# elucideye/acf

Measured on AMD Instinct MI355X. Metric: detector FPS @1080p, 8 scales/octave, FACE80 model, higher is better.
Workload: dtype f32

## Files before the change

### acf_amd/capi.py

```python
import ctypes as C
import os

import numpy as np

_HERE = os.path.dirname(os.path.abspath(__file__))
LIB_PATH = os.environ.get("ACF_HIP_LIB") or os.path.join(_HERE, "libacf_hip.so")

OK = 0
E_INVALID, E_UNSUPPORTED, E_NOMODEL, E_NOPLAN, E_HIP, E_NODEVICE, E_CAPACITY = 1, 2, 3, 4, 5, 6, 7
NMS_CAP = 2048
CS_GRAY, CS_RGB, CS_LUV, CS_HSV, CS_ORIG = 0, 1, 2, 3, 4
TAP_IMAGE, TAP_SMOOTHED, TAP_M, TAP_O, TAP_S, TAP_MNORM, TAP_CHNS, TAP_LDCF = range(8)


class Params(C.Structure):

    _fields_ = [
        ("nTrees", C.c_int32),
        ("nTreeNodes", C.c_int32),
        ("treeDepth", C.c_int32),
        ("fids", C.POINTER(C.c_uint32)),
        ("thrs", C.POINTER(C.c_float)),
        ("hs", C.POINTER(C.c_float)),
        ("child", C.POINTER(C.c_uint32)),
# ... 153 lines not shown
    fp = C.POINTER(C.c_float)
    sig = {
        "acf_hip_create": ([C.c_int, C.c_void_p, C.POINTER(ctx)], C.c_int),
        "acf_hip_destroy": ([ctx], C.c_int),
        "acf_hip_abi_version": ([], C.c_int),
        "acf_hip_device_count": ([C.POINTER(C.c_int)], C.c_int),
        "acf_hip_last_error": ([ctx], C.c_char_p),
        "acf_hip_set_option": ([ctx, C.c_char_p, C.c_int], C.c_int),
        "acf_hip_set_model": ([ctx, C.POINTER(Params)], C.c_int),
        "acf_hip_get_scales": ([C.c_int] * 7 + [C.POINTER(C.c_double)] * 3 + [C.c_int, C.POINTER(C.c_int)], C.c_int),
        "acf_hip_plan_levels": ([C.POINTER(Params), C.c_int, C.c_int, C.c_int, C.POINTER(Level), C.c_int, C.POINTER(C.c_int), C.POINTER(C.c_int)], C.c_int),
        "acf_hip_plan": ([ctx, C.c_int, C.c_int, C.c_int, C.c_int, C.c_int], C.c_int),
        "acf_hip_num_levels": ([ctx, C.POINTER(C.c_int), C.POINTER(C.c_int)], C.c_int),
        "acf_hip_get_levels": ([ctx, C.POINTER(Level), C.c_int], C.c_int),
        "acf_hip_get_ldcf_levels": ([ctx, C.POINTER(Level), C.c_int], C.c_int),
        "acf_hip_pyramid_floats": ([ctx, C.POINTER(C.c_int64)], C.c_int),
        "acf_hip_get_lambdas": ([ctx, C.c_int, C.POINTER(C.c_double)], C.c_int),
        "acf_hip_pyramid": ([ctx, C.c_void_p, C.c_int], C.c_int),
        "acf_hip_detect": ([ctx], C.c_int),
        "acf_hip_run": ([ctx, C.c_void_p, C.c_int], C.c_int),
        "acf_hip_run_host": ([ctx, fp, C.c_int], C.c_int),
        "acf_hip_pyramid_u8": ([ctx, C.c_void_p, C.c_int, C.c_int, C.c_int], C.c_int),
        "acf_hip_run_u8": ([ctx, C.c_void_p, C.c_int, C.c_int, C.c_int], C.c_int),
        "acf_hip_pyramid_image": ([ctx, C.c_void_p, C.c_int, C.POINTER(ImageDesc)], C.c_int),
        "acf_hip_run_image": ([ctx, C.c_void_p, C.c_int, C.POINTER(ImageDesc)], C.c_int),
        "acf_hip_image_extent": ([C.POINTER(ImageDesc), C.c_int, C.c_int, C.c_int, C.POINTER(C.c_int64), C.POINTER(C.c_int64)], C.c_int),
        "acf_hip_pyramid_yuv": ([ctx, C.c_void_p, C.c_int, C.POINTER(YuvDesc)], C.c_int),
        "acf_hip_run_yuv": ([ctx, C.c_void_p, C.c_int, C.POINTER(YuvDesc)], C.c_int),
        "acf_hip_yuv_to_rgb8": ([ctx, C.c_void_p, C.c_int, C.c_int, C.c_int, C.POINTER(YuvDesc), C.c_void_p], C.c_int),
        "acf_hip_yuv_extent": ([C.POINTER(YuvDesc), C.c_int, C.c_int, C.c_int, C.POINTER(C.c_int64), C.POINTER(C.c_int64)], C.c_int),
# ... 49 lines not shown
    return lib


DECLARED_SYMBOLS = [
    "acf_hip_create", "acf_hip_device_count", "acf_hip_destroy", "acf_hip_abi_version", "acf_hip_last_error", "acf_hip_set_option",
    "acf_hip_set_model", "acf_hip_get_scales", "acf_hip_plan_levels",
    "acf_hip_plan", "acf_hip_num_levels", "acf_hip_get_levels", "acf_hip_get_ldcf_levels", "acf_hip_pyramid_floats", "acf_hip_get_lambdas", "acf_hip_pyramid",
    "acf_hip_detect", "acf_hip_run", "acf_hip_run_host", "acf_hip_set_nms", "acf_hip_op_nms", "acf_hip_get_detections", "acf_hip_get_hits", "acf_hip_get_raw_detections",
    "acf_hip_pyramid_u8", "acf_hip_run_u8", "acf_hip_set_yuv_layout", "acf_hip_op_yuv420_to_rgb", "acf_hip_u8_frame_bytes", "acf_hip_resize_dims", "acf_hip_set_input_resize", "acf_hip_op_resize_u8", "acf_hip_stream_open", "acf_hip_stream_submit", "acf_hip_stream_collect",
    "acf_hip_stream_close", "acf_hip_host_alloc", "acf_hip_host_free",
    "acf_hip_export_detections", "acf_hip_synchronize", "acf_hip_get_repairs", "acf_hip_profile_get", "acf_hip_read_level", "acf_hip_read_rank_level", "acf_hip_rank_cells_host", "acf_hip_read_tap",
    "acf_hip_op_rgb_convert", "acf_hip_op_conv_tri", "acf_hip_op_gradient_mag", "acf_hip_selftest_gradmag", "acf_hip_set_x86_tables", "acf_hip_selftest_x86", "acf_hip_chns_compute", "acf_hip_op_gradient_hist",
    "acf_hip_op_im_resample", "acf_hip_op_acf_detect1", "acf_hip_op_acf_detect1_u8", "acf_hip_thrs_u8", "acf_hip_op_evaluate",
    "acf_hip_evaluate_crops", "acf_hip_evaluate_crops_u8",
    "acf_hip_pyramid_image", "acf_hip_run_image", "acf_hip_image_extent",
    "acf_hip_pyramid_yuv", "acf_hip_run_yuv", "acf_hip_yuv_to_rgb8", "acf_hip_yuv_extent", "acf_hip_yuv_layout", "acf_hip_stream_open_yuv",
]


def fptr(a):
    return a.ctypes.data_as(C.POINTER(C.c_float))
```

### acf_amd/csrc/acf_hip.hip

```cpp
#include "kernels.hip.h"

#include <algorithm>
#include <cmath>
#include <cstdio>
#include <cstring>
#include <functional>
#include <mutex>
#include <string>
#include <type_traits>
#include <vector>

using namespace acfhip;

namespace
{

struct DevBuf
{
    void* p = nullptr;
    size_t bytes = 0;
};

struct ResampleTiling
{
// ... 18 lines not shown
    StripPlan strip, stripPair;
    float *img = nullptr, *sm = nullptr, *M = nullptr, *O = nullptr, *U = nullptr, *S = nullptr, *Mn = nullptr;
    int64_t uFloats = 0, moFloats = 0;
};

}

struct TileSet
{
    bool ok = false;
    TileGeom g{};
    int nTiles = 0, aTB = 4;
    CascTile* d_tiles = nullptr;
    TreeNode* d_tileNodes = nullptr;
    uint32_t* d_tileNodesS = nullptr;
    uint32_t* d_nodesD = nullptr;
    int tbD = 0, t1D = 0;
    uint32_t* d_tileOffD = nullptr;
    uint32_t* d_thrsRankD = nullptr;
};

struct LeafCodes
{
    uint8_t* d = nullptr;
    int cap = 0, pitch = 0;
};

struct QueueCounters
{
    static constexpr size_t TILE_COUNTERS = 8;
// ... 260 lines not shown
{
    FB_TRIY_UNFUSED = 1u << 0,
    FB_MOU_PLAIN = 1u << 1,
    FB_RESAMPLE_NO_STRIP = 1u << 2,
    FB_RESAMPLE_NO_PAIR = 1u << 3,
    FB_RESAMPLE_NO_UP = 1u << 4,
    FB_RESAMPLE_GENERIC = 1u << 5,
    FB_LEVEL_GROUPS = 1u << 6,
    FB_LDCF_UNFUSED = 1u << 7,
    FB_NO_DEDUP = 1u << 8,
    FB_NO_TAIL_CODES = 1u << 9,
    FB_TAIL3 = 1u << 10,
    FB_TILED_STAGED = 1u << 11,
    FB_TILED_POOLED1 = 1u << 12,
    FB_YUV_UNFUSED = 1u << 13,
};
uint32_t fallbackMask()
{
    static const uint32_t mask = [] {
        static const struct { const char* name; uint32_t bit; } kNames[] = {
            { "triy_unfused", FB_TRIY_UNFUSED }, { "mou_plain", FB_MOU_PLAIN }, { "resample_no_strip", FB_RESAMPLE_NO_STRIP },
            { "resample_no_pair", FB_RESAMPLE_NO_PAIR }, { "resample_no_up", FB_RESAMPLE_NO_UP }, { "resample_generic", FB_RESAMPLE_GENERIC },
            { "level_groups", FB_LEVEL_GROUPS }, { "ldcf_unfused", FB_LDCF_UNFUSED }, { "no_dedup", FB_NO_DEDUP }, { "no_tail_codes", FB_NO_TAIL_CODES },
            { "tail3", FB_TAIL3 }, { "tiled_staged", FB_TILED_STAGED }, { "tiled_pooled1", FB_TILED_POOLED1 },
            { "yuv_unfused", FB_YUV_UNFUSED } };
        uint32_t m = 0;
        const char* e = getenv("ACF_HIP_FORCE_FALLBACK");
        std::string s = e ? e : "";
        size_t i = 0;
        while (i < s.size())
        {
            size_t j = s.find(',', i);
            j = j == std::string::npos ? s.size() : j;
            const std::string tok = s.substr(i, j - i);
            bool known = tok.empty();
            for (const auto& n : kNames)
            {
                if (tok == n.name)
                {
                    m |= n.bit;
// ... 1198 lines not shown
    }
    return ACF_HIP_OK;
}

int acf_hip_get_levels(const acf_hip_ctx* c, acf_hip_level* out, int cap)
{
    if (int rc = needPlanRead(c, "get_levels")) return rc;
    if (!out || cap < int(c->plan.levels.size()))
    {
        return fail(c, ACF_HIP_E_INVALID, "get_levels: capacity");
    }
    std::copy(c->plan.levels.begin(), c->plan.levels.end(), out);
    return ACF_HIP_OK;
}

int acf_hip_get_ldcf_levels(const acf_hip_ctx* c, acf_hip_level* out, int cap)
{
    if (!c || !c->hasPlan || !out)
    {
        return ACF_HIP_E_INVALID;
    }
    const acf_hip_ctx* src = c->kids.empty() ? c : c->kids[0];
    if (src->p.ldcfK <= 0 || src->ldcf.levels.empty())
    {
        return ACF_HIP_E_INVALID;
    }
    const int n = std::min(cap, int(src->ldcf.levels.size()));
    std::copy(src->ldcf.levels.begin(), src->ldcf.levels.begin() + n, out);
    return ACF_HIP_OK;
}
// ... 1266 lines not shown
```

### acf_amd/csrc/cascade_plan.hip.h

```cpp
#pragma once

struct FeatPos
{
    uint32_t z, cc, rr;
};

static inline FeatPos splitFid(uint32_t f, int mW, int mH)
{
    return { f / uint32_t(mW * mH), (f / uint32_t(mH)) % uint32_t(mW), f % uint32_t(mH) };
}

static size_t pooledTileLds(const TileGeom& g, int cellBytes, size_t leafBytes)
{
    const size_t nwin = size_t(g.NW) * 64;
    return leafBytes + size_t(g.tileFloats) * cellBytes + ((std::max(nwin * 8, size_t(g.passW) * size_t(g.pitchC)) + 15) / 16 * 16) + nwin * 8;
}

static int buildTileSet(acf_hip_ctx* c, const CascState& cs, const std::vector<float>& thrs, const std::vector<acf_hip_level>& lv, int nChns, const RankTables* rank,
    TileSet& out, bool allowPooledD = true)
{
    const acf_hip_params& p = c->p;
    const int mH = p.modelDsPad_h / cs.cell, mW = p.modelDsPad_w / cs.cell;
    const int cellBytes = rank ? 2 : 4, CPB = 16 / cellBytes;
    int rc;
// ... 95 lines not shown
    g.colsT = (g.TC - 1) * g.step + mW;
    g.rowsP = (g.rowsT + CPB - 1) / CPB * CPB;
    g.tileFloats = nChns * g.rowsP * g.colsT;
    g.cpsMagic = uint32_t(((uint64_t(1) << 32) + uint32_t(g.rowsP / CPB) - 1) / uint32_t(g.rowsP / CPB));
    g.colsMagic = uint32_t(((uint64_t(1) << 32) + uint32_t(g.colsT) - 1) / uint32_t(g.colsT));
    std::vector<CascTile> tiles;
    bool ok = true;
    {
        const uint32_t cps = uint32_t(g.rowsP / CPB), nSeg = uint32_t(nChns * g.colsT);
        for (uint32_t q = 0; q < nSeg * cps && ok; q++)
        {
            const uint32_t seg = uint32_t((uint64_t(q) * g.cpsMagic) >> 32);
            ok = seg == q / cps && uint32_t((uint64_t(seg) * g.colsMagic) >> 32) == seg / uint32_t(g.colsT);
        }
    }
    for (size_t i = 0; i < lv.size() && ok; i++)
    {
        for (int c0 = 0; c0 < lv[i].nWinC; c0 += g.TC)
        {
            for (int r0 = 0; r0 < lv[i].nWinR; r0 += g.TR)
            {
                if (r0 > 32767 || c0 > 32767)
                {
                    ok = false;
                    break;
                }
                CascTile t{};
                t.level = int16_t(i);
                t.r0 = int16_t(r0);
                t.c0 = int16_t(c0);
                tiles.push_back(t);
            }
        }
    }
    if (!ok)
    {
        return ACF_HIP_OK;
    }
    if (p.treeDepth != 2)
    {
        const int D = p.treeDepth;
        if ((rank && !g.pooled) || D < 1 || D > 4 || D == 2)
        {
            return ACF_HIP_OK;
        }
        const int NN = (1 << D) - 1, NL = 1 << D, TB = D == 1 ? 4 : (D == 3 ? 2 : 1);
        const int t1 = std::min(32, p.nTrees) / TB * TB;
// ... 48 lines not shown
            {
                return rc;
            }
        }
        out.g = g;
        out.nTiles = int(tiles.size());
        out.tbD = TB;
        out.t1D = t1;
        if ((rc = devUpload(c, &out.d_nodesD, nd)) || (rc = devUpload(c, &out.d_tiles, tiles)))
        {
            return rc;
        }
        out.ok = true;
        return ACF_HIP_OK;
    }
    std::vector<TreeNode> tileNodes(size_t(std::max(p.nTrees, 1)));
    for (int t = 0; t < p.nTrees; t++)
    {
        const size_t q = size_t(t) * p.nTreeNodes;
        TreeNode a{};
        for (int k = 0; k < 3; k++)
        {
            const FeatPos f = splitFid(c->fids[q + k], mW, mH);
            a.off[k] = (f.z * uint32_t(g.colsT) + f.cc) * uint32_t(g.rowsP) + f.rr;
            if (rank)
            {
                const uint32_t rk = rank->rankOfThreshold(int(f.z), thrs[q + k]);
                memcpy(&a.thr[k], &rk, 4);
            }
            else
            {
                a.thr[k] = thrs[q + k];
            }
        }
        for (int k = 0; k < 4; k++)
        {
            a.hs[k] = c->hs[q + 3 + k];
        }
        tileNodes[size_t(t)] = a;
    }
    const int aTB = 4;
    const int nTreesS = (g.pooled ? g.b[2] : g.b[1]) / aTB * aTB;
    std::vector<uint32_t> nodesS(size_t(std::max(nTreesS / aTB, 1)) * 10 * aTB, 0u);
    for (int t = 0; t + aTB - 1 < nTreesS; t += aTB)
    {
        uint32_t* d = nodesS.data() + size_t(t / aTB) * 10 * aTB;
        for (int q = 0; q < aTB; q++)
        {
            const TreeNode& nd = tileNodes[size_t(t + q)];
            for (int k = 0; k < 3; k++)
            {
                d[3 * q + k] = nd.off[k];
                memcpy(&d[3 * aTB + 3 * q + k], &nd.thr[k], 4);
            }
            for (int k = 0; k < 4; k++)
            {
                memcpy(&d[6 * aTB + 4 * q + k], &nd.hs[k], 4);
            }
        }
    }
    out.aTB = aTB;
    out.g = g;
    out.nTiles = int(tiles.size());
    if ((rc = devUpload(c, &out.d_tileNodesS, nodesS)) || (rc = devUpload(c, &out.d_tiles, tiles)) || (rc = devUpload(c, &out.d_tileNodes, tileNodes)))
    {
        return rc;
    }
    out.ok = true;
    return ACF_HIP_OK;
}

static LeafCodes leafCodeBuffer(acf_hip_ctx* c, const std::vector<acf_hip_level>& lv, int nT, int batch)
{
    LeafCodes lc;
    lc.pitch = (nT + 63) / 64 * 64;
    int64_t nWinTotal = 0;
    for (const auto& l : lv)
    {
// ... 357 lines not shown
```

### acf_amd/csrc/cascade_run.hip.h

```cpp
#pragma once

extern "C++"
{
template <class Args>
static int launchLds(acf_hip_ctx* c, void (*kernel)(Args), dim3 grid, dim3 block, size_t lds, const Args& a)
{
    int rc;
    if ((rc = allowLds(c, reinterpret_cast<const void*>(kernel), lds)))
    {
        return rc;
    }
    hipLaunchKernelGGL(kernel, grid, block, lds, c->stream, a);
    return ACF_HIP_OK;
}
}

using TileKernel = void (*)(TileArgs);
using TileDKernel = void (*)(TileDArgs);
using CascKernel = void (*)(CascArgs);

static TileKernel tile3Kernel(int nw, bool rank)
{
    if (rank)
    {
// ... 313 lines not shown
    {
        a.mH = c->p.modelDsPad_h / cs.cell;
        a.mW = c->p.modelDsPad_w / cs.cell;
    }
}
}

static void setTiles(TileArgs& a, const TileSet& ts)
{
    a.g = ts.g;
    a.tiles = ts.d_tiles;
    a.nTiles = ts.nTiles;
    a.tileNodes = ts.d_tileNodes;
    a.tileNodesS = ts.d_tileNodesS;
    a.aTB = ts.aTB;
}

static TileArgs tiled2Args(const acf_hip_ctx* c, const CascState& cs, const CascadeCall& call)
{
    const QueueCounters qc = cs.counters();
    TileArgs a{};
    fillShared(a, c, cs, call);
    setTiles(a, cs.tiles);
    a.nTrees = c->p.nTrees;
    a.tailNodes = cs.d_tailNodes;
    a.q = cs.d_queue[0];
    a.qcount = qc.queueCount();
    a.qhead = qc.queueHead();
    a.tileNext = qc.tileNext2();
    a.tailScratch = cs.d_tailScratch;
// ... 399 lines not shown
```

### acf_amd/csrc/host_plan.cpp

```cpp
#include "host_plan.h"

#include <algorithm>
#include <cfloat>
#include <cmath>
#include <cstring>
#include <limits>

namespace acfhip
{

ScaleList getScales(int nPerOct, int nOctUp, int minDs_h, int minDs_w, int shrink, int H, int W)
{
    ScaleList out;
    if (H <= 0 || W <= 0)
    {
        return out;
    }
    const double szw = H, szh = W;
    const double ratio_w = szw / double(minDs_h), ratio_h = szh / double(minDs_w);
    const double lg = std::log(std::min(ratio_w, ratio_h)) / std::log(2.0);
    const int nScales = int(std::floor(double(nPerOct) * (double(nOctUp) + lg) + 1.0));
    double d0 = szh, d1 = szw;
    if (szh >= szw)
    {
// ... 740 lines not shown
    {
        t.xlin[size_t(dx) * 4 + 3] = dx < xmax ? 1 : 0;
    }
    for (int dy = 0; dy < t.drows; dy++)
    {
        float f = float((dy + 0.5) * sc - 0.5);
        const int sy = cvFloorD(f);
        f -= sy;
        t.ylin[size_t(dy) * 4] = std::min(std::max(sy, 0), rows - 1);
        t.ylin[size_t(dy) * 4 + 1] = std::min(std::max(sy + 1, 0), rows - 1);
        t.ylin[size_t(dy) * 4 + 2] = satS16((1.f - f) * 2048.f);
        t.ylin[size_t(dy) * 4 + 3] = satS16(f * 2048.f);
    }
    return 0;
}
}
```

### acf_amd/csrc/host_plan.h

```cpp
#pragma once

#include "../../include/acf_hip.h"

#include <cstdint>
#include <string>
#include <vector>

namespace acfhip
{

struct ScaleList
{
    std::vector<double> scales, shw_h, shw_w;
};

ScaleList getScales(int nPerOct, int nOctUp, int minDs_h, int minDs_w, int shrink, int H, int W);

struct AxisCoef
{
    int na = 0, nb = 0;
    bool down = false;
    int bd[2] = { 0, 0 };
    std::vector<int> start;
    std::vector<int> src;
// ... 88 lines not shown
};

void buildRankTables(const float* thrs, const int32_t* chnOfNode, size_t nNodes, int nChns, RankTables& out);

struct ResizeTables
{
    int rows = 0, cols = 0, drows = 0, dcols = 0;
    int mode = 0, isx = 1, isy = 1;
    std::vector<int32_t> xlin, ylin;
    std::vector<int32_t> xrun, yrun;
    std::vector<int32_t> xtap, ytap;
};
void resizeDims(int rows, int cols, double scale, int& drows, int& dcols);
int buildResizeTables(int rows, int cols, double scale, ResizeTables& t);

int colorPlanes(const acf_hip_params& p);
int numChannels(const acf_hip_params& p);
int numChannels(const acf_hip_params& p, int dcol);

}
```

### acf_amd/csrc/kernels_cascade.hip.h

```cpp
#pragma once

namespace acfhip
{

struct CascLevel
{
    int32_t hP, wP, nWinR, nWinC;
    int32_t firstBlock;
    int32_t nWin;
    int64_t off;
    int64_t nodeOff;
    int64_t offR;
    int32_t pitchR;
    int32_t padR_;
};

struct __attribute__((aligned(16))) CascNode2
{
    uint32_t zcr[4];
    float thr[4];
    float hs[4];
};

struct CascArgs
// ... 476 lines not shown
            acf_hip_hit hit;
            hit.scale = lvl;
            hit.c = n / nWinR;
            hit.r = n - hit.c * nWinR;
            hit.score = h;
            a.hits[int64_t(frame) * a.maxHits + idx] = hit;
        }
    }
}

typedef uint32_t u32x4 __attribute__((ext_vector_type(4)));
typedef const __attribute__((address_space(4))) u32x4* cptr4_t;

struct CascTile
{
    int16_t level, pad_;
    int16_t r0, c0;
};

static_assert(sizeof(CascTile) == 8, "k_cascade_tile3 reads a CascTile as two dwords");
static_assert(offsetof(CascLevel, nWinR) == 8 && offsetof(CascLevel, off) == 24 && offsetof(CascLevel, offR) == 40 && offsetof(CascLevel, pitchR) == 48,
    "k_cascade_tile3 reads a CascLevel as dwords");

typedef const __attribute__((address_space(4))) uint32_t* cu32_k;
__device__ __forceinline__ CascTile load_tile_k(const CascTile* p)
{
    cu32_k tp = (cu32_k)(uintptr_t)p;
    const uint32_t w0 = tp[0], w1 = tp[1];
    CascTile T;
    T.level = int16_t(w0 & 0xffffu);
    T.pad_ = 0;
    T.r0 = int16_t(w1 & 0xffffu);
    T.c0 = int16_t(w1 >> 16);
    return T;
}
__device__ __forceinline__ CascLevel load_level_k(const CascLevel* p)
{
    cu32_k lp = (cu32_k)(uintptr_t)p;
    CascLevel L;
    L.hP = int32_t(lp[0]);
    L.wP = int32_t(lp[1]);
    L.nWinR = int32_t(lp[2]);
    L.nWinC = int32_t(lp[3]);
    L.off = int64_t(uint64_t(lp[6]) | (uint64_t(lp[7]) << 32));
    L.offR = int64_t(uint64_t(lp[10]) | (uint64_t(lp[11]) << 32));
    L.pitchR = int32_t(lp[12]);
// ... 8 lines not shown
};

struct TileGeom
{
    int32_t TR, TC, NW, W;
    int32_t step;
    int32_t rowsT, colsT;
    int32_t rowsP;
    int32_t tileFloats;
    uint32_t cpsMagic, colsMagic;
    int32_t b[5];
    int32_t winFloats;
    int32_t pooled;
    int32_t passW;
    int32_t pitchC;
};

struct TileArgs
{
    const float* pyr;
    int64_t pyr_fs;
    const uint16_t* pyrR;
    int64_t pyrR_fs;
    const CascLevel* levels;
    const CascTile* tiles;
    int32_t nTiles, nFrames, nChns, mH, mW, nTrees;
    TileGeom g;
    const TreeNode* tileNodes;
    const uint32_t* tileNodesS;
    int32_t aTB;
// ... 2 lines not shown
    uint2* q;
    int32_t* qcount;
    int32_t* qhead;
    int32_t* tileNext;
    int32_t qcap;
    acf_hip_hit* hits;
    int32_t* counts;
    int32_t maxHits;
    int32_t debug;
    long long* stamps;
    float* tailScratch;
    int32_t tailPad, tailSlab;
    int32_t tailNodesLds;
    uint8_t* tailCodes;
    int32_t codeCap, codePitch;
};

struct LaneNode
{
    uint4 o, tq, hq;
};

#ifdef ACF_HIP_STAMPS
#define TILE_STAMP(k)                                                          \
    if ((a.debug & 4) && threadIdx.x == 0)                                      \
    {                                                                          \
        a.stamps[int64_t(blockIdx.x) * 8 + (k)] = __builtin_amdgcn_s_memtime(); \
    }
#else
#define TILE_STAMP(k)
// ... 221 lines not shown
    }
    alive = alive && (hMin > thrC);
}

template <int NW, class CT>
__global__ void __launch_bounds__(NW * 64) k_cascade_tile3(TileArgs a)
{
    typedef typename CT::cell_t cell_t;
    typedef typename CT::val_t val_t;
    constexpr int CPB = CT::CPB;
    constexpr int NT = NW * 64;
    extern __shared__ float lds[];
    __shared__ int s_n[4];
    float* leafT = lds;
    cell_t* tileF = reinterpret_cast<cell_t*>(reinterpret_cast<char*>(lds) + TILE3_LEAF_BYTES);
    const int NWIN = a.g.TR * a.g.TC;
    char* r1 = reinterpret_cast<char*>(tileF) + size_t(a.g.tileFloats) * sizeof(cell_t);
    const int passW = a.g.passW;
    const int r1Bytes = (max(NWIN * 8, passW * a.g.pitchC) + 15) & ~15;
    uint2* l1 = reinterpret_cast<uint2*>(r1);
    uint8_t* codes = reinterpret_cast<uint8_t*>(r1);
    uint2* l2 = reinterpret_cast<uint2*>(r1 + r1Bytes);
    const int tid = threadIdx.x, lane = tid & 63, wv = tid >> 6;

    const int64_t total = int64_t(a.nTiles) * a.nFrames;
    const int perX = int((total + 7) >> 3);
    const int xcd = blockIdx.x & 7;
    __shared__ int s_next[2];
    const bool persist = a.tileNext != nullptr;
    int li = int(blockIdx.x >> 3);
    if (persist)
    {
        if (tid == 0)
        {
            s_next[0] = atomicAdd(a.tileNext + xcd, 1);
        }
        __syncthreads();
        li = __builtin_amdgcn_readfirstlane(s_next[0]);
    }
    int par = 1;
    const int step = a.g.step, rowsP = a.g.rowsP, TR = a.g.TR;
    const int b1 = a.g.b[1], b2 = a.g.b[2], tEnd = a.g.b[4];
    const int Ts = tEnd - b2, TsPad = (Ts + 15) & ~15;
    const int tlShift = TsPad <= 32 ? 5 : (TsPad <= 64 ? 6 : 7);
    const int pos = tid & ((1 << tlShift) - 1);
    uint32_t so0 = 0, so1 = 0, so2 = 0, st0 = 0, st1 = 0, st2 = 0;
    if (Ts > 0)
    {
        const uint4* np = reinterpret_cast<const uint4*>(a.tileNodes + b2 + min(pos, Ts - 1));
        const uint4 o = np[0], tq = np[1];
        so0 = o.x, so1 = o.y, so2 = o.z;
        st0 = tq.x, st1 = tq.y, st2 = tq.z;
    }
    bool leavesDone = Ts <= 0;
    for (;;)
    {
    const int64_t id = int64_t(xcd) * perX + li;
    if (li >= perX || id >= total)
    {
        break;
    }
    int liNext = perX;
    if (tid == 0 && persist)
    {
        liNext = atomicAdd(a.tileNext + xcd, 1);
    }
    const int frame = int(id / a.nTiles);
    const CascTile T = load_tile_k(a.tiles + (id - int64_t(frame) * a.nTiles));
    const int lvl = T.level;
    const CascLevel L = load_level_k(a.levels + lvl);
    const int nWinR = L.nWinR;
    if (tid < 4)
    {
        s_n[tid] = 0;
    }
    TILE_STAMP(0);
    {
        const int colsT = a.g.colsT;
        const int gr0 = T.r0 * step, gc0 = T.c0 * step;
        const int colPitch = CT::RANK ? L.pitchR : L.hP;
        const int area = colPitch * L.wP;
        const cell_t* __restrict__ src0 = (CT::RANK ? reinterpret_cast<const cell_t*>(a.pyrR) + int64_t(frame) * a.pyrR_fs + L.offR
                                                    : reinterpret_cast<const cell_t*>(a.pyr) + int64_t(frame) * a.pyr_fs + L.off) + gr0;
        const srd_t fsrd = make_srd(src0, int64_t(a.nChns) * area * int64_t(sizeof(cell_t)));
        const int colsValid = min(colsT, L.wP - gc0);
        const uint32_t cps = uint32_t(rowsP) / uint32_t(CPB);
        const uint32_t nChunks = uint32_t(a.nChns * colsT) * cps;
        const int ccMax = colsValid - 1;
        for (uint32_t q0 = uint32_t(wv) * 64u; q0 < nChunks; q0 += NW * 64u)
        {
            const uint32_t q = q0 + lane;
            if (q < nChunks)
            {
                const uint32_t seg = __umulhi(q, a.g.cpsMagic);
                const uint32_t j = q - seg * cps;
                const uint32_t z = __umulhi(seg, a.g.colsMagic);
                const int cc = int(seg - z * uint32_t(colsT));
                const uint32_t soff = z * uint32_t(area) + uint32_t(gc0 + min(cc, ccMax)) * uint32_t(colPitch) + uint32_t(CPB) * j;
                __builtin_amdgcn_raw_ptr_buffer_load_lds(fsrd, (lptr_t)(tileF + uint32_t(CPB) * q0), 16, soff * uint32_t(sizeof(cell_t)), 0, 0, 0);
            }
        }
    }
    const int r_l = lane % TR, c_l = (lane / TR) * NW + wv;
    const bool aliveA1 = (T.r0 + r_l) < nWinR && (T.c0 + c_l) < L.nWinC && lane < (64 / TR) * TR;
    if (!leavesDone)
    {
        for (int t = tid; t < TsPad; t += NT)
        {
            float4 hv = make_float4(-0.f, -0.f, -0.f, -0.f);
            if (t < Ts)
            {
                hv = *reinterpret_cast<const float4*>(a.tileNodes[b2 + t].hs);
            }
            leafT[4 * t] = hv.x;
            leafT[4 * t + 1] = hv.y;
            leafT[4 * t + 2] = hv.z;
// ... 42 lines not shown
            if (lane == 0)
            {
                base = atomicAdd(cnt, __popcll(m));
            }
            base = __shfl(base, 0);
            if (alive)
            {
                list[base + __popcll(m & ((1ull << lane) - 1ull))] = make_uint2(__float_as_uint(h), tw);
            }
        }
    };
    auto dense = [&](const cell_t* win, int t0, int t1, float& h, bool& alive) {
        const int nb = (t1 - t0) / 4;
        if (nb > 0)
        {
            tile_eval_p<CT>(win, a.tileNodesS + size_t(t0 / 4) * 40, nb, thrC, h, alive);
        }
        tile_eval_s1<CT>(win, a.tileNodes, t0 + nb * 4, t1, thrC, h, alive);
    };

    {
        bool alive = aliveA1;
        float h = 0.f;
        const uint32_t woff = uint32_t((min(c_l, a.g.TC - 1) * step) * rowsP + r_l * step);
        dense(tileF + woff, 0, b1, h, alive);
        const uint32_t tw = uint32_t(c_l * TR + r_l) | (woff << 16);
        if (b1 == tEnd)
        {
            finish((tile_args_k)__builtin_amdgcn_kernarg_segment_ptr(), alive, tw, h);
        }
        else
        {
            append(alive, tw, h, b1 == b2 ? l2 : l1, b1 == b2 ? &s_n[1] : &s_n[0]);
        }
    }
    TILE_STAMP(2);
    __syncthreads();
    TILE_STAMP(3);
    tile_args_k ak = (tile_args_k)__builtin_amdgcn_kernarg_segment_ptr();
    asm volatile("" : "+s"(ak));
// ... 157 lines not shown
    par ^= 1;
    if (!wantE)
    {
        continue;
    }
    const int nTail = s_n[3];
#ifdef ACF_HIP_STAMPS
    if ((a.debug & 4) && threadIdx.x == 0)
    {
        a.stamps[int64_t(blockIdx.x) * 8 + 7] = (long long)s_n[0] | ((long long)s_n[1] << 16) | ((long long)nTail << 32);
    }
#endif
    if (nTail != 0)
    {
        const int nTrees = ak->nTrees, codeCap = ak->codeCap, codePitch = ak->codePitch;
        const TreeNode* __restrict__ nodes = ak->tileNodes + tEnd;
        uint8_t* __restrict__ codesG = ak->tailCodes + int64_t(frame) * codeCap * codePitch + lane;
        const int nT = nTrees - tEnd, nB = (nT + 63) >> 6;
        for (int b0 = wv; b0 < nB; b0 += 4 * NW)
        {
            uint32_t o0[4], o1[4], o2[4];
            val_t t0[4], t1[4], t2[4];
#pragma unroll
            for (int k = 0; k < 4; k++)
            {
                const int b = min(b0 + k * NW, nB - 1);
                const uint4* np = reinterpret_cast<const uint4*>(nodes + min(b * 64 + lane, nT - 1));
                const uint4 o = np[0], tq = np[1];
                o0[k] = o.x;
                o1[k] = o.y;
                o2[k] = o.z;
// ... 1242 lines not shown
```

### include/acf_hip.h

```cpp
#ifndef ACF_HIP_H
#define ACF_HIP_H

#include <stddef.h>
#include <stdint.h>

#ifdef __cplusplus
extern "C" {
#endif

#define ACF_HIP_ABI_VERSION 9

#if defined(__GNUC__)
#define ACF_HIP_API __attribute__((visibility("default")))
#else
#define ACF_HIP_API
#endif

enum {
    ACF_HIP_OK = 0,
    ACF_HIP_E_INVALID = 1,
    ACF_HIP_E_UNSUPPORTED = 2,
    ACF_HIP_E_NOMODEL = 3,
    ACF_HIP_E_NOPLAN = 4,
    ACF_HIP_E_HIP = 5,
// ... 101 lines not shown
ACF_HIP_API int acf_hip_set_option(acf_hip_ctx* ctx, const char* key, int value);

ACF_HIP_API int acf_hip_set_x86_tables(acf_hip_ctx* ctx, const uint32_t* rcp4096, const uint32_t* rsqrt8192);
ACF_HIP_API int acf_hip_selftest_x86(acf_hip_ctx* ctx, uint32_t first_bits, uint64_t count, uint32_t stride, uint64_t digest[3]);

ACF_HIP_API int acf_hip_get_scales(int nPerOct, int nOctUp, int minDs_h, int minDs_w, int shrink, int h, int w,
    double* scales, double* scaleshw_h, double* scaleshw_w, int cap, int* n);

ACF_HIP_API int acf_hip_plan_levels(const acf_hip_params* p, int h, int w, int d, acf_hip_level* out, int cap, int* nScales, int* nChns);

ACF_HIP_API int acf_hip_set_model(acf_hip_ctx* ctx, const acf_hip_params* p);

ACF_HIP_API int acf_hip_plan(acf_hip_ctx* ctx, int h, int w, int d, int max_batch, int max_hits);
ACF_HIP_API int acf_hip_num_levels(const acf_hip_ctx* ctx, int* nScales, int* nChns);
ACF_HIP_API int acf_hip_get_levels(const acf_hip_ctx* ctx, acf_hip_level* out, int cap);
ACF_HIP_API int acf_hip_get_ldcf_levels(const acf_hip_ctx* ctx, acf_hip_level* out, int cap);
ACF_HIP_API int acf_hip_pyramid_floats(const acf_hip_ctx* ctx, int64_t* n);
ACF_HIP_API int acf_hip_get_lambdas(acf_hip_ctx* ctx, int frame, double out[3]);


ACF_HIP_API int acf_hip_pyramid(acf_hip_ctx* ctx, const float* frames_dev, int n_frames);

ACF_HIP_API int acf_hip_detect(acf_hip_ctx* ctx);

ACF_HIP_API int acf_hip_run(acf_hip_ctx* ctx, const float* frames_dev, int n_frames);

ACF_HIP_API int acf_hip_run_host(acf_hip_ctx* ctx, const float* frames_host, int n_frames);

enum {
    ACF_HIP_PIX_RGB = 0,
// ... 129 lines not shown
```

Before: 16450.

## Tile cascade windows with up to four row-height shapes chosen per level

Instead of one fixed tile shape (TR×TC windows) for every pyramid level, the planner now uses dynamic programming to pick up to four tile shapes with the same per-tile LDS footprint. Each level's rows are split into bands so that fewer, better-filled tiles cover the window grid. Per-shape feature offsets are baked into duplicated node tables, and the tiled kernel reads the shape from the tile descriptor through kernarg. It also skips the dense stage when no lane in a wave is alive. The cost is more node memory, extra per-tile kernarg loads, and reloading stage nodes when the shape changes between tiles.

```diff
diff --git a/acf_amd/capi.py b/acf_amd/capi.py
--- a/acf_amd/capi.py
+++ b/acf_amd/capi.py
@@ -191,6 +191,9 @@
         "acf_hip_num_levels": ([ctx, C.POINTER(C.c_int), C.POINTER(C.c_int)], C.c_int),
         "acf_hip_get_levels": ([ctx, C.POINTER(Level), C.c_int], C.c_int),
         "acf_hip_get_ldcf_levels": ([ctx, C.POINTER(Level), C.c_int], C.c_int),
+        "acf_hip_get_tile_bands": ([ctx, C.c_int, C.POINTER(C.c_int32), C.c_int, C.POINTER(C.c_int), C.POINTER(C.c_int32)], C.c_int),
+        "acf_hip_tile_bands_host": ([C.POINTER(C.c_int32), C.POINTER(C.c_int32), C.c_int, C.POINTER(C.c_int32), C.POINTER(C.c_int32), C.POINTER(C.c_int32),
+                                     C.c_int, C.POINTER(C.c_int), C.POINTER(C.c_int64)], C.c_int),
         "acf_hip_pyramid_floats": ([ctx, C.POINTER(C.c_int64)], C.c_int),
         "acf_hip_get_lambdas": ([ctx, C.c_int, C.POINTER(C.c_double)], C.c_int),
         "acf_hip_pyramid": ([ctx, C.c_void_p, C.c_int], C.c_int),
@@ -270,6 +273,7 @@
     "acf_hip_op_im_resample", "acf_hip_op_acf_detect1", "acf_hip_op_acf_detect1_u8", "acf_hip_thrs_u8", "acf_hip_op_evaluate",
     "acf_hip_evaluate_crops", "acf_hip_evaluate_crops_u8",
     "acf_hip_pyramid_image", "acf_hip_run_image", "acf_hip_image_extent",
+    "acf_hip_get_tile_bands", "acf_hip_tile_bands_host",
     "acf_hip_pyramid_yuv", "acf_hip_run_yuv", "acf_hip_yuv_to_rgb8", "acf_hip_yuv_extent", "acf_hip_yuv_layout", "acf_hip_stream_open_yuv",
 ]
 
diff --git a/acf_amd/csrc/acf_hip.hip b/acf_amd/csrc/acf_hip.hip
--- a/acf_amd/csrc/acf_hip.hip
+++ b/acf_amd/csrc/acf_hip.hip
@@ -56,6 +56,10 @@
     CascTile* d_tiles = nullptr;
     TreeNode* d_tileNodes = nullptr;
     uint32_t* d_tileNodesS = nullptr;
+    int nShapes = 1;
+    TileShape sh[TILE3_MAX_SHAPES] = {};
+    std::vector<TileBand> bands;
+    int nTilesOne = 0;
     uint32_t* d_nodesD = nullptr;
     int tbD = 0, t1D = 0;
     uint32_t* d_tileOffD = nullptr;
@@ -346,6 +350,7 @@
     FB_TILED_STAGED = 1u << 11,
     FB_TILED_POOLED1 = 1u << 12,
     FB_YUV_UNFUSED = 1u << 13,
+    FB_TILE_SHAPE_ONE = 1u << 14,
 };
 uint32_t fallbackMask()
 {
@@ -355,7 +360,7 @@
             { "resample_no_pair", FB_RESAMPLE_NO_PAIR }, { "resample_no_up", FB_RESAMPLE_NO_UP }, { "resample_generic", FB_RESAMPLE_GENERIC },
             { "level_groups", FB_LEVEL_GROUPS }, { "ldcf_unfused", FB_LDCF_UNFUSED }, { "no_dedup", FB_NO_DEDUP }, { "no_tail_codes", FB_NO_TAIL_CODES },
             { "tail3", FB_TAIL3 }, { "tiled_staged", FB_TILED_STAGED }, { "tiled_pooled1", FB_TILED_POOLED1 },
-            { "yuv_unfused", FB_YUV_UNFUSED } };
+            { "yuv_unfused", FB_YUV_UNFUSED }, { "tile_shape_one", FB_TILE_SHAPE_ONE } };
         uint32_t m = 0;
         const char* e = getenv("ACF_HIP_FORCE_FALLBACK");
         std::string s = e ? e : "";
@@ -1584,6 +1589,66 @@
     return ACF_HIP_OK;
 }
 
+int acf_hip_get_tile_bands(const acf_hip_ctx* c, int rank_cells, int32_t* bands, int cap, int* n, int32_t* info)
+{
+    if (!c || !c->hasPlan || !n || !info || (cap > 0 && !bands))
+    {
+        return ACF_HIP_E_INVALID;
+    }
+    const acf_hip_ctx* src = c->kids.empty() ? c : c->kids[0];
+    const TileSet& ts = rank_cells ? src->cs.tilesR : src->cs.tiles;
+    if (src->p.treeDepth != 2 || !ts.ok)
+    {
+        return ACF_HIP_E_INVALID;
+    }
+    *n = int(ts.bands.size());
+    for (int i = 0; i < std::min(cap, *n); i++)
+    {
+        bands[3 * i] = ts.bands[size_t(i)].level;
+        bands[3 * i + 1] = ts.bands[size_t(i)].r0;
+        bands[3 * i + 2] = ts.sh[ts.bands[size_t(i)].shape].TR;
+    }
+    info[0] = ts.nShapes;
+    info[1] = ts.nTiles;
+    info[2] = ts.nTilesOne;
+    info[3] = ts.sh[0].TR;
+    return ACF_HIP_OK;
+}
+
+int acf_hip_tile_bands_host(const int32_t* nWinR, const int32_t* nWinC, int nLevels, const int32_t* geom, int32_t* shapes, int32_t* bands, int cap, int* n,
+    int64_t* tiles)
+{
+    if (!nWinR || !nWinC || nLevels < 0 || !geom || !shapes || !n || !tiles || (cap > 0 && !bands) || (geom[6] != 2 && geom[6] != 4) || geom[7] < 1 ||
+        geom[7] > TILE3_MAX_SHAPES)
+    {
+        return ACF_HIP_E_INVALID;
+    }
+    TileShapePlan sp;
+    chooseTileShapes(nWinR, nWinC, nLevels, geom[0], geom[1], geom[2], geom[3], geom[4], geom[5], 16 / geom[6], geom[7], sp);
+    if (sp.shapes.empty() || sp.shapes[0].TR <= 0)
+    {
+        return ACF_HIP_E_INVALID;
+    }
+    for (int k = 0; k < geom[7]; k++)
+    {
+        const TileShapeGeom g = size_t(k) < sp.shapes.size() ? sp.shapes[size_t(k)] : TileShapeGeom{};
+        shapes[4 * k] = g.TR;
+        shapes[4 * k + 1] = g.TC;
+        shapes[4 * k + 2] = g.colsT;
+        shapes[4 * k + 3] = g.rowsP;
+    }
+    *n = int(sp.bands.size());
+    for (int i = 0; i < std::min(cap, *n); i++)
+    {
+        bands[3 * i] = sp.bands[size_t(i)].level;
+        bands[3 * i + 1] = sp.bands[size_t(i)].r0;
+        bands[3 * i + 2] = sp.bands[size_t(i)].shape;
+    }
+    tiles[0] = sp.tilesOne;
+    tiles[1] = sp.tiles;
+    return ACF_HIP_OK;
+}
+
 int acf_hip_get_ldcf_levels(const acf_hip_ctx* c, acf_hip_level* out, int cap)
 {
     if (!c || !c->hasPlan || !out)
diff --git a/acf_amd/csrc/cascade_plan.hip.h b/acf_amd/csrc/cascade_plan.hip.h
--- a/acf_amd/csrc/cascade_plan.hip.h
+++ b/acf_amd/csrc/cascade_plan.hip.h
@@ -133,23 +133,35 @@
             ok = seg == q / cps && uint32_t((uint64_t(seg) * g.colsMagic) >> 32) == seg / uint32_t(g.colsT);
         }
     }
-    for (size_t i = 0; i < lv.size() && ok; i++)
-    {
-        for (int c0 = 0; c0 < lv[i].nWinC; c0 += g.TC)
-        {
-            for (int r0 = 0; r0 < lv[i].nWinR; r0 += g.TR)
-            {
-                if (r0 > 32767 || c0 > 32767)
-                {
-                    ok = false;
-                    break;
-                }
-                CascTile t{};
-                t.level = int16_t(i);
-                t.r0 = int16_t(r0);
-                t.c0 = int16_t(c0);
-                tiles.push_back(t);
-            }
+    TileShapePlan sp;
+    {
+        std::vector<int32_t> wr(lv.size()), wc(lv.size());
+        for (size_t i = 0; i < lv.size(); i++)
+        {
+            wr[i] = lv[i].nWinR;
+            wc[i] = lv[i].nWinC;
+        }
+        const bool mixed = p.treeDepth == 2 && !getenv("ACF_HIP_TILE_TR") && !nwEnv && !fallbackForced(FB_TILE_SHAPE_ONE);
+        chooseTileShapes(wr.data(), wc.data(), int(lv.size()), g.TR, g.NW, g.step, mH, mW, nChns, CPB, mixed ? TILE3_MAX_SHAPES : 1, sp);
+    }
+    ok = ok && !sp.shapes.empty() && sp.shapes[0].TR == g.TR && sp.shapes[0].TC == g.TC;
+    for (size_t i = 0; i < sp.bands.size() && ok; i++)
+    {
+        const TileBand& bd = sp.bands[i];
+        const TileShapeGeom& sg = sp.shapes[size_t(bd.shape)];
+        for (int c0 = 0; c0 < lv[size_t(bd.level)].nWinC; c0 += sg.TC)
+        {
+            if (bd.r0 > 32767 || c0 > 32767)
+            {
+                ok = false;
+                break;
+            }
+            CascTile t{};
+            t.level = int16_t(bd.level);
+            t.shape = int16_t(bd.shape);
+            t.r0 = int16_t(bd.r0);
+            t.c0 = int16_t(c0);
+            tiles.push_back(t);
         }
     }
     if (!ok)
@@ -228,15 +240,18 @@
         out.ok = true;
         return ACF_HIP_OK;
     }
-    std::vector<TreeNode> tileNodes(size_t(std::max(p.nTrees, 1)));
-    for (int t = 0; t < p.nTrees; t++)
-    {
-        const size_t q = size_t(t) * p.nTreeNodes;
+    const int nShapes = int(sp.shapes.size());
+    const size_t nodesPer = size_t(std::max(p.nTrees, 1));
+    std::vector<TreeNode> tileNodes(nodesPer * nShapes);
+    for (int t = 0; t < p.nTrees * nShapes; t++)
+    {
+        const TileShapeGeom& sg = sp.shapes[size_t(t / p.nTrees)];
+        const size_t q = size_t(t % p.nTrees) * p.nTreeNodes;
         TreeNode a{};
         for (int k = 0; k < 3; k++)
         {
             const FeatPos f = splitFid(c->fids[q + k], mW, mH);
-            a.off[k] = (f.z * uint32_t(g.colsT) + f.cc) * uint32_t(g.rowsP) + f.rr;
+            a.off[k] = (f.z * uint32_t(sg.colsT) + f.cc) * uint32_t(sg.rowsP) + f.rr;
             if (rank)
             {
                 const uint32_t rk = rank->rankOfThreshold(int(f.z), thrs[q + k]);
@@ -251,31 +266,43 @@
         {
             a.hs[k] = c->hs[q + 3 + k];
         }
-        tileNodes[size_t(t)] = a;
+        tileNodes[size_t(t / p.nTrees) * nodesPer + size_t(t % p.nTrees)] = a;
     }
     const int aTB = 4;
     const int nTreesS = (g.pooled ? g.b[2] : g.b[1]) / aTB * aTB;
-    std::vector<uint32_t> nodesS(size_t(std::max(nTreesS / aTB, 1)) * 10 * aTB, 0u);
-    for (int t = 0; t + aTB - 1 < nTreesS; t += aTB)
-    {
-        uint32_t* d = nodesS.data() + size_t(t / aTB) * 10 * aTB;
-        for (int q = 0; q < aTB; q++)
-        {
-            const TreeNode& nd = tileNodes[size_t(t + q)];
-            for (int k = 0; k < 3; k++)
-            {
-                d[3 * q + k] = nd.off[k];
-                memcpy(&d[3 * aTB + 3 * q + k], &nd.thr[k], 4);
-            }
-            for (int k = 0; k < 4; k++)
-            {
-                memcpy(&d[6 * aTB + 4 * q + k], &nd.hs[k], 4);
+    const size_t nodesSPer = size_t(std::max(nTreesS / aTB, 1)) * 10 * aTB;
+    std::vector<uint32_t> nodesS(nodesSPer * nShapes, 0u);
+    for (int si = 0; si < nShapes; si++)
+    {
+        for (int t = 0; t + aTB - 1 < nTreesS; t += aTB)
+        {
+            uint32_t* d = nodesS.data() + si * nodesSPer + size_t(t / aTB) * 10 * aTB;
+            for (int q = 0; q < aTB; q++)
+            {
+                const TreeNode& nd = tileNodes[si * nodesPer + size_t(t + q)];
+                for (int k = 0; k < 3; k++)
+                {
+                    d[3 * q + k] = nd.off[k];
+                    memcpy(&d[3 * aTB + 3 * q + k], &nd.thr[k], 4);
+                }
+                for (int k = 0; k < 4; k++)
+                {
+                    memcpy(&d[6 * aTB + 4 * q + k], &nd.hs[k], 4);
+                }
             }
         }
     }
     out.aTB = aTB;
     out.g = g;
     out.nTiles = int(tiles.size());
+    out.nShapes = nShapes;
+    out.bands = sp.bands;
+    out.nTilesOne = int(sp.tilesOne);
+    for (int si = 0; si < nShapes; si++)
+    {
+        const TileShapeGeom& sg = sp.shapes[size_t(si)];
+        out.sh[si] = TileShape{ sg.TR, sg.TC, sg.colsT, sg.rowsP, sg.cpsMagic, sg.colsMagic, int32_t(si * nodesPer), int32_t(si * nodesSPer) };
+    }
     if ((rc = devUpload(c, &out.d_tileNodesS, nodesS)) || (rc = devUpload(c, &out.d_tiles, tiles)) || (rc = devUpload(c, &out.d_tileNodes, tileNodes)))
     {
         return rc;
diff --git a/acf_amd/csrc/cascade_run.hip.h b/acf_amd/csrc/cascade_run.hip.h
--- a/acf_amd/csrc/cascade_run.hip.h
+++ b/acf_amd/csrc/cascade_run.hip.h
@@ -351,6 +351,10 @@
     a.tileNodes = ts.d_tileNodes;
     a.tileNodesS = ts.d_tileNodesS;
     a.aTB = ts.aTB;
+    for (int i = 0; i < TILE3_MAX_SHAPES; i++)
+    {
+        a.sh[i] = ts.sh[i < ts.nShapes ? i : 0];
+    }
 }
 
 static TileArgs tiled2Args(const acf_hip_ctx* c, const CascState& cs, const CascadeCall& call)
diff --git a/acf_amd/csrc/host_plan.cpp b/acf_amd/csrc/host_plan.cpp
--- a/acf_amd/csrc/host_plan.cpp
+++ b/acf_amd/csrc/host_plan.cpp
@@ -778,4 +778,122 @@
     }
     return 0;
 }
-}
+
+TileShapeGeom tileShapeGeom(int TR, int NW, int step, int mH, int mW, int nChns, int CPB)
+{
+    TileShapeGeom s;
+    if (TR < 1 || TR > 64 || NW < 1 || step < 1 || mH < 1 || mW < 1 || nChns < 1 || CPB < 1)
+    {
+        return s;
+    }
+    s.TR = TR;
+    s.TC = (64 / TR) * NW;
+    s.rowsT = (TR - 1) * step + mH;
+    s.colsT = (s.TC - 1) * step + mW;
+    s.rowsP = (s.rowsT + CPB - 1) / CPB * CPB;
+    s.cells = int64_t(nChns) * s.colsT * s.rowsP;
+    const uint32_t cps = uint32_t(s.rowsP / CPB), nSeg = uint32_t(nChns) * uint32_t(s.colsT);
+    s.cpsMagic = uint32_t(((uint64_t(1) << 32) + cps - 1) / cps);
+    s.colsMagic = uint32_t(((uint64_t(1) << 32) + uint32_t(s.colsT) - 1) / uint32_t(s.colsT));
+    s.magicOk = s.cells < (int64_t(1) << 24);
+    for (uint32_t q = 0; s.magicOk && q < nSeg * cps; q++)
+    {
+        const uint32_t seg = uint32_t((uint64_t(q) * s.cpsMagic) >> 32);
+        s.magicOk = seg == q / cps && uint32_t((uint64_t(seg) * s.colsMagic) >> 32) == seg / uint32_t(s.colsT);
+    }
+    return s;
+}
+
+static int64_t bandsOfLevel(int nWinR, int nWinC, const std::vector<TileShapeGeom>& sh, std::vector<int32_t>* bands)
+{
+    if (nWinR <= 0 || nWinC <= 0)
+    {
+        return 0;
+    }
+    std::vector<int64_t> f(size_t(nWinR) + 1, 0);
+    std::vector<int32_t> pick(size_t(nWinR) + 1, 0);
+    for (int r = 1; r <= nWinR; r++)
+    {
+        int64_t best = -1;
+        for (size_t k = 0; k < sh.size(); k++)
+        {
+            const int64_t n = f[size_t(std::max(r - sh[k].TR, 0))] + (nWinC + sh[k].TC - 1) / sh[k].TC;
+            if (best < 0 || n < best)
+            {
+                best = n;
+                pick[size_t(r)] = int32_t(k);
+            }
+        }
+        f[size_t(r)] = best;
+    }
+    for (int r = nWinR; bands && r > 0; r -= sh[size_t(pick[size_t(r)])].TR)
+    {
+        bands->push_back(pick[size_t(r)]);
+    }
+    return f[size_t(nWinR)];
+}
+
+void chooseTileShapes(const int32_t* nWinR, const int32_t* nWinC, int nLevels, int TR0, int NW, int step, int mH, int mW, int nChns, int CPB, int maxShapes,
+    TileShapePlan& out)
+{
+    out = TileShapePlan{};
+    out.shapes.push_back(tileShapeGeom(TR0, NW, step, mH, mW, nChns, CPB));
+    if (out.shapes[0].TR <= 0)
+    {
+        return;
+    }
+    const int64_t cells0 = out.shapes[0].cells;
+    std::vector<TileShapeGeom> cand;
+    for (int tr = 8; tr <= 64; tr++)
+    {
+        const TileShapeGeom s = tileShapeGeom(tr, NW, step, mH, mW, nChns, CPB);
+        if (tr != TR0 && (64 / tr) * tr >= 48 && s.cells <= cells0 && s.magicOk)
+        {
+            cand.push_back(s);
+        }
+    }
+    auto total = [&](const std::vector<TileShapeGeom>& sh) {
+        int64_t n = 0;
+        for (int i = 0; i < nLevels; i++)
+        {
+            n += bandsOfLevel(nWinR[i], nWinC[i], sh, nullptr);
+        }
+        return n;
+    };
+    out.tilesOne = total(out.shapes);
+    out.tiles = out.tilesOne;
+    while (int(out.shapes.size()) < maxShapes)
+    {
+        int pick = -1;
+        int64_t bestN = out.tiles;
+        for (size_t k = 0; k < cand.size(); k++)
+        {
+            std::vector<TileShapeGeom> sh = out.shapes;
+            sh.push_back(cand[k]);
+            const int64_t n = total(sh);
+            if (n < bestN)
+            {
+                bestN = n;
+                pick = int(k);
+            }
+        }
+        if (pick < 0)
+        {
+            break;
+        }
+        out.shapes.push_back(cand[size_t(pick)]);
+        out.tiles = bestN;
+    }
+    for (int i = 0; i < nLevels; i++)
+    {
+        std::vector<int32_t> b;
+        bandsOfLevel(nWinR[i], nWinC[i], out.shapes, &b);
+        int r0 = 0;
+        for (int32_t k : b)
+        {
+            out.bands.push_back({ int32_t(i), int32_t(r0), k });
+            r0 += out.shapes[size_t(k)].TR;
+        }
+    }
+}
+}
diff --git a/acf_amd/csrc/host_plan.h b/acf_amd/csrc/host_plan.h
--- a/acf_amd/csrc/host_plan.h
+++ b/acf_amd/csrc/host_plan.h
@@ -126,6 +126,28 @@
 void resizeDims(int rows, int cols, double scale, int& drows, int& dcols);
 int buildResizeTables(int rows, int cols, double scale, ResizeTables& t);
 
+struct TileShapeGeom
+{
+    int TR = 0, TC = 0, rowsT = 0, colsT = 0, rowsP = 0;
+    int64_t cells = 0;
+    uint32_t cpsMagic = 0, colsMagic = 0;
+    bool magicOk = false;
+};
+TileShapeGeom tileShapeGeom(int TR, int NW, int step, int mH, int mW, int nChns, int CPB);
+
+struct TileBand
+{
+    int32_t level, r0, shape;
+};
+struct TileShapePlan
+{
+    std::vector<TileShapeGeom> shapes;
+    std::vector<TileBand> bands;
+    int64_t tilesOne = 0, tiles = 0;
+};
+void chooseTileShapes(const int32_t* nWinR, const int32_t* nWinC, int nLevels, int TR0, int NW, int step, int mH, int mW, int nChns, int CPB, int maxShapes,
+    TileShapePlan& out);
+
 int colorPlanes(const acf_hip_params& p);
 int numChannels(const acf_hip_params& p);
 int numChannels(const acf_hip_params& p, int dcol);
diff --git a/acf_amd/csrc/kernels_cascade.hip.h b/acf_amd/csrc/kernels_cascade.hip.h
--- a/acf_amd/csrc/kernels_cascade.hip.h
+++ b/acf_amd/csrc/kernels_cascade.hip.h
@@ -514,7 +514,7 @@
 
 struct CascTile
 {
-    int16_t level, pad_;
+    int16_t level, shape;
     int16_t r0, c0;
 };
 
@@ -529,7 +529,7 @@
     const uint32_t w0 = tp[0], w1 = tp[1];
     CascTile T;
     T.level = int16_t(w0 & 0xffffu);
-    T.pad_ = 0;
+    T.shape = int16_t(w0 >> 16);
     T.r0 = int16_t(w1 & 0xffffu);
     T.c0 = int16_t(w1 >> 16);
     return T;
@@ -568,6 +568,15 @@
     int32_t pooled;
     int32_t passW;
     int32_t pitchC;
+};
+
+#define TILE3_MAX_SHAPES 4
+struct TileShape
+{
+    int32_t TR, TC;
+    int32_t colsT, rowsP;
+    uint32_t cpsMagic, colsMagic;
+    int32_t nodeOff, nodeOffS;
 };
 
 struct TileArgs
@@ -600,6 +609,7 @@
     int32_t tailNodesLds;
     uint8_t* tailCodes;
     int32_t codeCap, codePitch;
+    TileShape sh[TILE3_MAX_SHAPES];
 };
 
 struct LaneNode
@@ -851,7 +861,7 @@
     __shared__ int s_n[4];
     float* leafT = lds;
     cell_t* tileF = reinterpret_cast<cell_t*>(reinterpret_cast<char*>(lds) + TILE3_LEAF_BYTES);
-    const int NWIN = a.g.TR * a.g.TC;
+    constexpr int NWIN = NT;
     char* r1 = reinterpret_cast<char*>(tileF) + size_t(a.g.tileFloats) * sizeof(cell_t);
     const int passW = a.g.passW;
     const int r1Bytes = (max(NWIN * 8, passW * a.g.pitchC) + 15) & ~15;
@@ -876,19 +886,13 @@
         li = __builtin_amdgcn_readfirstlane(s_next[0]);
     }
     int par = 1;
-    const int step = a.g.step, rowsP = a.g.rowsP, TR = a.g.TR;
+    const int step = a.g.step;
     const int b1 = a.g.b[1], b2 = a.g.b[2], tEnd = a.g.b[4];
     const int Ts = tEnd - b2, TsPad = (Ts + 15) & ~15;
     const int tlShift = TsPad <= 32 ? 5 : (TsPad <= 64 ? 6 : 7);
     const int pos = tid & ((1 << tlShift) - 1);
     uint32_t so0 = 0, so1 = 0, so2 = 0, st0 = 0, st1 = 0, st2 = 0;
-    if (Ts > 0)
-    {
-        const uint4* np = reinterpret_cast<const uint4*>(a.tileNodes + b2 + min(pos, Ts - 1));
-        const uint4 o = np[0], tq = np[1];
-        so0 = o.x, so1 = o.y, so2 = o.z;
-        st0 = tq.x, st1 = tq.y, st2 = tq.z;
-    }
+    int nodeShape = -1;
     bool leavesDone = Ts <= 0;
     for (;;)
     {
@@ -907,13 +911,18 @@
     const int lvl = T.level;
     const CascLevel L = load_level_k(a.levels + lvl);
     const int nWinR = L.nWinR;
+    const __attribute__((address_space(4))) TileShape* shp = &((tile_args_k)__builtin_amdgcn_kernarg_segment_ptr())->sh[T.shape];
+    const int TR = shp->TR, TC = shp->TC, rowsP = shp->rowsP;
+    const TreeNode* __restrict__ tileNodes = a.tileNodes + shp->nodeOff;
+    const uint32_t* __restrict__ tileNodesS = a.tileNodesS + shp->nodeOffS;
     if (tid < 4)
     {
         s_n[tid] = 0;
     }
     TILE_STAMP(0);
     {
-        const int colsT = a.g.colsT;
+        const int colsT = shp->colsT;
+        const uint32_t cpsMagic = shp->cpsMagic, colsMagic = shp->colsMagic;
         const int gr0 = T.r0 * step, gc0 = T.c0 * step;
         const int colPitch = CT::RANK ? L.pitchR : L.hP;
         const int area = colPitch * L.wP;
@@ -929,14 +938,22 @@
             const uint32_t q = q0 + lane;
             if (q < nChunks)
             {
-                const uint32_t seg = __umulhi(q, a.g.cpsMagic);
+                const uint32_t seg = __umulhi(q, cpsMagic);
                 const uint32_t j = q - seg * cps;
-                const uint32_t z = __umulhi(seg, a.g.colsMagic);
+                const uint32_t z = __umulhi(seg, colsMagic);
                 const int cc = int(seg - z * uint32_t(colsT));
                 const uint32_t soff = z * uint32_t(area) + uint32_t(gc0 + min(cc, ccMax)) * uint32_t(colPitch) + uint32_t(CPB) * j;
                 __builtin_amdgcn_raw_ptr_buffer_load_lds(fsrd, (lptr_t)(tileF + uint32_t(CPB) * q0), 16, soff * uint32_t(sizeof(cell_t)), 0, 0, 0);
             }
         }
+    }
+    if (Ts > 0 && nodeShape != T.shape)
+    {
+        const uint4* np = reinterpret_cast<const uint4*>(tileNodes + b2 + min(pos, Ts - 1));
+        const uint4 o = np[0], tq = np[1];
+        so0 = o.x, so1 = o.y, so2 = o.z;
+        st0 = tq.x, st1 = tq.y, st2 = tq.z;
+        nodeShape = T.shape;
     }
     const int r_l = lane % TR, c_l = (lane / TR) * NW + wv;
     const bool aliveA1 = (T.r0 + r_l) < nWinR && (T.c0 + c_l) < L.nWinC && lane < (64 / TR) * TR;
@@ -1009,16 +1026,19 @@
         const int nb = (t1 - t0) / 4;
         if (nb > 0)
         {
-            tile_eval_p<CT>(win, a.tileNodesS + size_t(t0 / 4) * 40, nb, thrC, h, alive);
-        }
-        tile_eval_s1<CT>(win, a.tileNodes, t0 + nb * 4, t1, thrC, h, alive);
+            tile_eval_p<CT>(win, tileNodesS + size_t(t0 / 4) * 40, nb, thrC, h, alive);
+        }
+        tile_eval_s1<CT>(win, tileNodes, t0 + nb * 4, t1, thrC, h, alive);
     };
 
     {
         bool alive = aliveA1;
         float h = 0.f;
-        const uint32_t woff = uint32_t((min(c_l, a.g.TC - 1) * step) * rowsP + r_l * step);
-        dense(tileF + woff, 0, b1, h, alive);
+        const uint32_t woff = uint32_t((min(c_l, TC - 1) * step) * rowsP + r_l * step);
+        if (__ballot(aliveA1) != 0ull)
+        {
+            dense(tileF + woff, 0, b1, h, alive);
+        }
         const uint32_t tw = uint32_t(c_l * TR + r_l) | (woff << 16);
         if (b1 == tEnd)
         {
@@ -1206,7 +1226,7 @@
     if (nTail != 0)
     {
         const int nTrees = ak->nTrees, codeCap = ak->codeCap, codePitch = ak->codePitch;
-        const TreeNode* __restrict__ nodes = ak->tileNodes + tEnd;
+        const TreeNode* __restrict__ nodes = ak->tileNodes + ak->sh[T.shape].nodeOff + tEnd;
         uint8_t* __restrict__ codesG = ak->tailCodes + int64_t(frame) * codeCap * codePitch + lane;
         const int nT = nTrees - tEnd, nB = (nT + 63) >> 6;
         for (int b0 = wv; b0 < nB; b0 += 4 * NW)
diff --git a/include/acf_hip.h b/include/acf_hip.h
--- a/include/acf_hip.h
+++ b/include/acf_hip.h
@@ -139,6 +139,9 @@
 ACF_HIP_API int acf_hip_plan(acf_hip_ctx* ctx, int h, int w, int d, int max_batch, int max_hits);
 ACF_HIP_API int acf_hip_num_levels(const acf_hip_ctx* ctx, int* nScales, int* nChns);
 ACF_HIP_API int acf_hip_get_levels(const acf_hip_ctx* ctx, acf_hip_level* out, int cap);
+ACF_HIP_API int acf_hip_get_tile_bands(const acf_hip_ctx* ctx, int rank_cells, int32_t* bands, int cap, int* n, int32_t* info);
+ACF_HIP_API int acf_hip_tile_bands_host(const int32_t* nWinR, const int32_t* nWinC, int nLevels, const int32_t* geom, int32_t* shapes, int32_t* bands,
+    int cap, int* n, int64_t* tiles);
 ACF_HIP_API int acf_hip_get_ldcf_levels(const acf_hip_ctx* ctx, acf_hip_level* out, int cap);
 ACF_HIP_API int acf_hip_pyramid_floats(const acf_hip_ctx* ctx, int64_t* n);
 ACF_HIP_API int acf_hip_get_lambdas(acf_hip_ctx* ctx, int frame, double out[3]);
```

Measured after the change: 16590 (median of 6 runs). No clear change (+0.8%).
